# microsoft/foldingdiff

Hardware: AMD Instinct MI355X
Metric: backbones/sec (L=128, T=1000, bs=512) (higher is better)
Workload: dtype f32 (fp16 hi/lo split operands, 3x v_mfma_f32_{32x32x16,16x16x32}_f16 per product, fp32 accumulate)

## Files before the change

foldingdiff_amd/csrc/ffn16.hip:

```cpp
#include <cstdlib>
#include <type_traits>

#include "fdmi_kernels.h"
#include "img_common.h"
#include "launch_common.h"

namespace fdmi {
namespace ffn {

typedef float f32x4 __attribute__((ext_vector_type(4)));
typedef const __attribute__((address_space(3))) u32x4* lds_cu128_t;
__device__ __forceinline__ unsigned lds_addr(const void* p) { return (unsigned)(unsigned long long)(lds_ptr_t)(const_cast<void*>(p)); }
__device__ __forceinline__ u32x4 lds_u128(unsigned a) { return *(lds_cu128_t)(unsigned long long)a; }
__device__ __forceinline__ f16x8 lds_f16x8(unsigned a) { return __builtin_bit_cast(f16x8, lds_u128(a)); }

__device__ __forceinline__ void swap16(unsigned& vdst, unsigned& src) {
  const auto r = __builtin_amdgcn_permlane16_swap(vdst, src, false, false);
  vdst = r[0];
  src = r[1];
}
__device__ __forceinline__ float quad_sum(float x) {
  unsigned a = __builtin_bit_cast(unsigned, x), b = a;
  swap32(a, b);
  float m = __builtin_bit_cast(float, a) + __builtin_bit_cast(float, b);
  a = __builtin_bit_cast(unsigned, m);
  b = a;
  swap16(a, b);
  return __builtin_bit_cast(float, a) + __builtin_bit_cast(float, b);
}

template <int V> using IC = std::integral_constant<int, V>;
template <int LO, int HI, class F>
__device__ __forceinline__ void static_for(F&& f) {
  if constexpr (LO < HI) {
    f(IC<LO>{});
    static_for<LO + 1, HI>(f);
  }
}

#ifndef FDMI_FFN_DBG
#define FDMI_FFN_DBG 0
#endif
#ifndef FDMI_FFN_ST_AUX
#define FDMI_FFN_ST_AUX 0
#endif
#ifndef FDMI_FFN_PRIO
#define FDMI_FFN_PRIO 2
#endif

__device__ __forceinline__ f32x4 mfma16(const f16x8& a, const f16x8& b, const f32x4& c) {
  return __builtin_amdgcn_mfma_f32_16x16x32_f16(a, b, c, 0, 0, 0);
}

constexpr int NW = 8;
constexpr int TILE = 2048;
constexpr int STEP = 4 * TILE;
constexpr int SPS = 2;
constexpr int STAGE = SPS * STEP;
constexpr int NST = 3;
constexpr int PPW = STAGE / 1024 / NW;
constexpr int OFF_W = 0;
constexpr int OFF_X = NST * STAGE;
__host__ __device__ constexpr int off_p(int nkt) { return OFF_X + NW * nkt * 1024; }

template <int NKT, bool TAIL, bool PROF>
__global__ __launch_bounds__(64 * NW) void ffn16_kernel(FfnArgs p) {
  static_assert(NKT == 12 || NKT == 6, "d_model 384 or 192, intermediate size 2 d_model");
  constexpr int D = 32 * NKT;
  constexpr int NG = NKT;
  constexpr int SPG = 2 * NKT;
  constexpr int STG = SPG / SPS;
  static_assert(STG % NST == 0, "a group is a whole number of ring turns: its first stage always sits in slot 0");
  constexpr int NSA = TAIL ? NKT * NKT / 2 : 0;
  static_assert((NSA / SPS) % NST == 0 && NSA % SPS == 0, "whole ring turns");
  constexpr int W_BYTES = (NSA / SPS + NG * STG) * STAGE;
  constexpr int OFF_P = off_p(NKT);
  constexpr int OFF_P1 = OFF_P + 5 * D * 4;
  extern __shared__ __attribute__((aligned(16))) unsigned char smem[];
  const int tid = threadIdx.x, lane = tid & 63;
  const int wq = __builtin_amdgcn_readfirstlane(tid >> 6);
  const int grp = wq >> 2;
  unsigned smem0 = __builtin_amdgcn_readfirstlane(lds_addr(smem));
  asm volatile("" : "+s"(smem0));
  auto lane_id = [&]() __attribute__((always_inline)) {
    int ln;
    asm volatile("v_mbcnt_lo_u32_b32 %0, -1, 0\n\tv_mbcnt_hi_u32_b32 %0, -1, %0" : "=v"(ln));
    return ln;
  };
  auto lane_off_of = [](int ln) __attribute__((always_inline)) { return (unsigned)((ln >> 4) * 256 + (ln & 15) * 16); };

  {
    float* par = reinterpret_cast<float*>(smem + OFF_P);
    for (int i = tid; i < 2 * D; i += 64 * NW) par[i] = p.bi[i];
    for (int i = tid; i < D; i += 64 * NW) {
      par[2 * D + i] = p.bd[i];
      par[3 * D + i] = p.gamma[i];
      par[4 * D + i] = p.beta[i] * p.out_scale;
      if constexpr (TAIL) {
        par[5 * D + i] = p.bo[i] * (1.0f / p.ao_scale);
        par[6 * D + i] = p.g1[i];
        par[7 * D + i] = p.b1[i] * p.a_scale;
      }
    }
  }

  int w_src = 0, w_slot = 0;
  const __amdgpu_buffer_rsrc_t rs_w = __builtin_amdgcn_make_buffer_rsrc(const_cast<unsigned char*>(p.wimg), 0, W_BYTES, 0x00020000);
  auto issue_w = [&]() __attribute__((always_inline)) {
    const lds_ptr_t dst = (lds_ptr_t)(unsigned long long)(smem0 + OFF_W + (unsigned)__builtin_amdgcn_readfirstlane(w_slot));
    const int so = __builtin_amdgcn_readfirstlane(w_src);
    const int vo = lane_id() * 16;
#pragma unroll
    for (int k = 0; k < PPW; ++k) dma16(rs_w, dst + (wq + NW * k) * 1024, vo, so + (wq + NW * k) * 1024);
    w_src = w_src + STAGE == W_BYTES ? 0 : w_src + STAGE;
    w_slot = w_slot + STAGE == NST * STAGE ? 0 : w_slot + STAGE;
  };

  f16x8 ah[NKT];
  const __amdgpu_buffer_rsrc_t rs_a =
      __builtin_amdgcn_make_buffer_rsrc(const_cast<unsigned char*>(TAIL ? p.cimg : p.aimg), 0, p.a_bytes, 0x00020000);
  const __amdgpu_buffer_rsrc_t rs_h = __builtin_amdgcn_make_buffer_rsrc(const_cast<unsigned char*>(TAIL ? p.hres : p.aimg), 0, p.a_bytes, 0x00020000);
  auto row_off = [&](int r0) __attribute__((always_inline)) {
    const int ln = lane_id();
    const int row = r0 + 16 * wq + (ln & 15);
    return (unsigned)(((row >> 5) * (NKT * 256) + (row & 31)) * 16 + (ln >> 4) * 512);
  };
  u32x4 tl[NKT];
  auto load_hi = [&](int r0) __attribute__((always_inline)) {
    const unsigned hoff = row_off(r0);
#pragma unroll
    for (int kt = 0; kt < NKT; ++kt)
      ah[kt] = __builtin_bit_cast(f16x8, __builtin_amdgcn_raw_buffer_load_b128(rs_a, (int)hoff, kt * 8 * 512, 0));
  };
  auto load_lo = [&](auto KT, unsigned hoff) __attribute__((always_inline)) {
    constexpr int kt = decltype(KT)::value;
    tl[kt] = __builtin_bit_cast(u32x4, __builtin_amdgcn_raw_buffer_load_b128(rs_a, (int)hoff, (kt * 8 + 4) * 512, 0));
  };
  auto commit_lo = [&]() __attribute__((always_inline)) {
    const unsigned ax = smem0 + OFF_X + (unsigned)(wq * NKT * 1024 + lane_id() * 16);
#pragma unroll
    for (int kt = 0; kt < NKT; ++kt) *(__attribute__((address_space(3))) u32x4*)(unsigned long long)(ax + (unsigned)(kt * 1024)) = tl[kt];
  };
  const __amdgpu_buffer_rsrc_t rs_o = __builtin_amdgcn_make_buffer_rsrc(p.out, 0, p.out_bytes, 0x00020000);
  auto load_res = [&](auto KT, unsigned hoff, f32x4 (&Yr)[2 * NKT]) __attribute__((always_inline)) {
    constexpr int kt = decltype(KT)::value;
    Yr[2 * kt] = __builtin_bit_cast(f32x4, __builtin_amdgcn_raw_buffer_load_b128(rs_h, (int)hoff, kt * 8 * 512, 0));
    Yr[2 * kt + 1] = __builtin_bit_cast(f32x4, __builtin_amdgcn_raw_buffer_load_b128(rs_h, (int)hoff, (kt * 8 + 4) * 512, 0));
  };

  const bool rec = PROF && blockIdx.x == 0 && p.stamps != nullptr;
  unsigned long long* stp = PROF ? p.stamps + (size_t)wq * 16 * 16 : nullptr;
  int slot = 0;
#define FD_STAMP(i) do { if (PROF) { if (rec && slot < 16 && lane == 0) stp[slot * 16 + (i)] = __builtin_amdgcn_s_memtime(); } } while (0)
#define FD_SB() __builtin_amdgcn_sched_barrier(0)
#define FD_STAMP_G(i) do { if (PROF) { if (rec && slot == 0 && G == 1 && lane == 0) stp[15 * 16 + (i)] = __builtin_amdgcn_s_memtime(); } } while (0)

  const int n_pass = p.dims ? min(p.panels, __builtin_amdgcn_readfirstlane(p.dims[1]) >> 7) : p.panels;
  if ((int)blockIdx.x >= n_pass) return;
  const float os_up = p.up_scale, os_dn = p.down_scale, hs = 0.5f * p.g_scale;
  const f32x4 zero4 = {0.f, 0.f, 0.f, 0.f};
  f32x4 Y[2 * NKT];
  f32x4 U[4];
  f32x4 Up[4];
  u32x4 uh[2], ul[2];

  load_hi((int)blockIdx.x * 128);
  {
    const unsigned hoff = row_off((int)blockIdx.x * 128);
    static_for<0, NKT>([&](auto KT) __attribute__((always_inline)) { load_lo(KT, hoff); });
    if constexpr (TAIL) static_for<0, NKT>([&](auto KT) __attribute__((always_inline)) { load_res(KT, hoff, Y); });
  }
  issue_w();
  issue_w();
  issue_w();
  FD_WAIT_VM(3 * PPW);
  commit_lo();
  FD_WAIT_VM(2 * PPW);
  barrier_keep_vm();

  auto gelu_piece = [&](auto P, unsigned abq) __attribute__((always_inline)) {
    constexpr int pc = decltype(P)::value, pr = pc >> 2, j = pc & 3;
    const u32x2 b = *(const __attribute__((address_space(3))) u32x2*)(unsigned long long)(abq + (unsigned)((32 * pr + 2 * j) * 4));
    float o0 = __builtin_fmaf(Up[2 * pr + (j >> 1)][2 * (j & 1)], os_up, __builtin_bit_cast(float, (unsigned)b[0]));
    float o1 = __builtin_fmaf(Up[2 * pr + (j >> 1)][2 * (j & 1) + 1], os_up, __builtin_bit_cast(float, (unsigned)b[1]));
#if !(FDMI_FFN_DBG & 1)
    const float h0 = o0 * hs, h1 = o1 * hs;
    o0 = __builtin_fmaf(h0, erf_rational(o0 * 0.70710678118654752440f), h0);
    o1 = __builtin_fmaf(h1, erf_rational(o1 * 0.70710678118654752440f), h1);
#endif
    unsigned a, c;
    split_pair(o0, o1, a, c);
    uh[pr][j] = a;
    ul[pr][j] = c;
  };

  auto steps = [&](auto S0, auto S1, auto GEL, unsigned abq) __attribute__((always_inline)) {
    constexpr int s0 = decltype(S0)::value, s1 = decltype(S1)::value;
    constexpr bool gel = decltype(GEL)::value == 1, pha = decltype(GEL)::value == 2;
    auto stage_top = [&]() __attribute__((always_inline)) {
      FD_WAIT_VM(PPW);
      barrier_keep_vm();
      issue_w();
    };
    f16x8 fx[4], fy[4], xl;
    unsigned a_W, a_X;
    {
      const int ln = lane_id();
      a_W = smem0 + OFF_W + lane_off_of(ln);
      a_X = smem0 + OFF_X + (unsigned)(wq * NKT * 1024 + ln * 16);
      asm volatile("" : "+v"(a_W), "+v"(a_X));
    }
    auto plane_reads = [&](auto S, auto LO, f16x8 (&f)[4]) __attribute__((always_inline)) {
      constexpr int s = decltype(S)::value, lo = decltype(LO)::value;
      constexpr unsigned off = (unsigned)(((s / SPS) % NST) * STAGE + (s % SPS) * STEP + lo * 1024);
#if FDMI_FFN_DBG & 8
      if constexpr (lo == 1) {
#pragma unroll
        for (int t = 0; t < 4; ++t) f[t] = fx[t];
      } else
#endif
#pragma unroll
      for (int t = 0; t < 4; ++t) f[t] = lds_f16x8(a_W + off + (unsigned)(t * TILE));
      if constexpr (pha) {
        if constexpr (lo == 0 && s % (NKT / 2) == 0) xl = lds_f16x8(a_X + (unsigned)((s / (NKT / 2)) * 1024));
      } else {
        if constexpr (lo == 0 && s < NKT) xl = lds_f16x8(a_X + (unsigned)(s * 1024));
      }
    };
    auto mm = [&](auto S, auto WHICH, const f16x8 (&f)[4]) __attribute__((always_inline)) {
      constexpr int s = decltype(S)::value, which = decltype(WHICH)::value;
      if constexpr (pha) {
        constexpr int kt = s / (NKT / 2), q = s % (NKT / 2);
#pragma unroll
        for (int t = 0; t < 4; ++t) Y[4 * q + t] = mfma16(f[t], which == 1 ? xl : ah[kt], Y[4 * q + t]);
      } else if constexpr (s < NKT) {
#if !(FDMI_FFN_DBG & 4)
#pragma unroll
        for (int t = 0; t < 4; ++t) U[t] = mfma16(f[t], which == 1 ? xl : ah[s], U[t]);
#endif
      } else {
#if !(FDMI_FFN_DBG & 2)
        constexpr int pr = (s - NKT) / (NKT / 2), q = (s - NKT) % (NKT / 2);
#pragma unroll
        for (int t = 0; t < 4; ++t) Y[4 * q + t] = mfma16(f[t], __builtin_bit_cast(f16x8, which == 1 ? ul[pr] : uh[pr]), Y[4 * q + t]);
#endif
      }
    };
    plane_reads(S0, IC<0>{}, fx);
    FD_SB();
    static_for<s0, s1>([&](auto S) __attribute__((always_inline)) {
      constexpr int s = decltype(S)::value;
      constexpr bool top = s % SPS == SPS - 1;
      plane_reads(S, IC<1>{}, fy);
      FD_SB();
      if constexpr (top) {
        if (grp == 0) stage_top();
      }
#if FDMI_FFN_PRIO
      __builtin_amdgcn_s_setprio(FDMI_FFN_PRIO);
#endif
      mm(S, IC<0>{}, fx);
      mm(S, IC<1>{}, fx);
#if FDMI_FFN_PRIO
      __builtin_amdgcn_s_setprio(0);
#endif
      FD_SB();
      if constexpr (top) {
        if (grp != 0) stage_top();
      }
      if constexpr (s + 1 < s1) plane_reads(IC<s + 1>{}, IC<0>{}, fx);
      FD_SB();
      if constexpr (gel) {
        if (grp == 0) {
          static_for<0, 8>([&](auto P) __attribute__((always_inline)) {
            if constexpr (1 + decltype(P)::value * (NKT - 2) / 8 == s) gelu_piece(P, abq);
          });
        }
        FD_SB();
      }
      mm(S, IC<2>{}, fy);
      FD_SB();
      if constexpr (gel) {
        if (grp != 0) {
          static_for<0, 8>([&](auto P) __attribute__((always_inline)) {
            if constexpr (1 + decltype(P)::value * (NKT - 2) / 8 == s) gelu_piece(P, abq);
          });
        }
        FD_SB();
      }
    });
  };

  for (int panel = blockIdx.x; panel < n_pass; panel += (int)gridDim.x) {
    FD_STAMP(0);
    if constexpr (TAIL) {
      const int ln = lane_id();
      const int g = ln >> 4;
      const unsigned pb1 = smem0 + OFF_P1 + (unsigned)(8 * g * 4);
      const unsigned ax = smem0 + OFF_X + (unsigned)(wq * NKT * 1024 + ln * 16);
      {
        const float c = p.hres_inv * (1.0f / p.ao_scale);
#pragma unroll
        for (int kt = 0; kt < NKT; ++kt) {
          const u32x4 rh = __builtin_bit_cast(u32x4, Y[2 * kt]), rl = __builtin_bit_cast(u32x4, Y[2 * kt + 1]);
          const u32x4 b0 = lds_u128(pb1 + (unsigned)(kt * 128)), b1 = lds_u128(pb1 + (unsigned)(kt * 128 + 16));
#pragma unroll
          for (int j = 0; j < 2; ++j)
#pragma unroll
            for (int e = 0; e < 4; e += 2) {
              const unsigned hw = rh[2 * j + e / 2], lw = rl[2 * j + e / 2];
              const unsigned bw0 = j == 0 ? b0[e] : b1[e], bw1 = j == 0 ? b0[e + 1] : b1[e + 1];
              float v0 = fma_mix_lo(hw, c, __builtin_bit_cast(float, bw0));
              float v1 = fma_mix_hi(hw, c, __builtin_bit_cast(float, bw1));
              Y[2 * kt + j][e] = fma_mix_lo(lw, c, v0);
              Y[2 * kt + j][e + 1] = fma_mix_hi(lw, c, v1);
            }
        }
      }
      steps(IC<0>{}, IC<NSA>{}, IC<2>{}, 0u);
      const float os_ao = p.ao_scale;
      float sum = 0.f;
#pragma unroll
      for (int t = 0; t < 2 * NKT; ++t)
#pragma unroll
        for (int e = 0; e < 4; ++e) {
          Y[t][e] *= os_ao;
          sum += Y[t][e];
        }
      const float inv_n = 1.0f / (float)D;
      float mean = quad_sum(sum) * inv_n;
      asm volatile("" : "+v"(mean));
      float t2 = 0.f;
#pragma unroll
      for (int t = 0; t < 2 * NKT; ++t)
#pragma unroll
        for (int e = 0; e < 4; ++e) {
          const float dl = Y[t][e] - mean;
          Y[t][e] = dl;
          t2 = __builtin_fmaf(dl, dl, t2);
        }
      const float rstd = (1.0f / sqrtf(__builtin_fmaf(quad_sum(t2), inv_n, p.eps1))) * p.a_scale;
#pragma unroll
      for (int kt = 0; kt < NKT; ++kt) {
        const u32x4 g0 = lds_u128(pb1 + (unsigned)(D * 4 + kt * 128)), g1 = lds_u128(pb1 + (unsigned)(D * 4 + kt * 128 + 16));
        const u32x4 e0 = lds_u128(pb1 + (unsigned)(2 * D * 4 + kt * 128)), e1 = lds_u128(pb1 + (unsigned)(2 * D * 4 + kt * 128 + 16));
        float o[8];
#pragma unroll
        for (int e = 0; e < 4; ++e) {
          o[e] = __builtin_fmaf(Y[2 * kt][e] * rstd, __builtin_bit_cast(float, (unsigned)g0[e]), __builtin_bit_cast(float, (unsigned)e0[e]));
          o[4 + e] = __builtin_fmaf(Y[2 * kt + 1][e] * rstd, __builtin_bit_cast(float, (unsigned)g1[e]), __builtin_bit_cast(float, (unsigned)e1[e]));
        }
        u32x4 hv, lv;
#pragma unroll
        for (int j = 0; j < 4; ++j) {
          unsigned a, b;
          split_pair(o[2 * j], o[2 * j + 1], a, b);
          hv[j] = a;
          lv[j] = b;
        }
        ah[kt] = __builtin_bit_cast(f16x8, hv);
        *(__attribute__((address_space(3))) u32x4*)(unsigned long long)(ax + (unsigned)(kt * 1024)) = lv;
      }
    }
#pragma unroll
    for (int t = 0; t < 2 * NKT; ++t) Y[t] = zero4;
#pragma unroll
    for (int t = 0; t < 4; ++t) U[t] = zero4;
    steps(IC<0>{}, IC<NKT>{}, IC<0>{}, 0u);
    for (int G = 0; G < NG; ++G) {
#pragma unroll
      for (int t = 0; t < 4; ++t) {
        Up[t] = U[t];
        U[t] = zero4;
      }
      unsigned abq = smem0 + OFF_P + (unsigned)((64 * G + 8 * (lane_id() >> 4)) * 4);
      asm volatile("" : "+v"(abq));
      FD_STAMP_G(0);
      FD_STAMP_G(1);
      if (G + 1 < NG) {
#ifdef FDMI_FFN_NOPIPE
        static_for<0, 8>([&](auto P) __attribute__((always_inline)) { gelu_piece(P, abq); });
        steps(IC<0>{}, IC<NKT>{}, IC<0>{}, abq);
#else
        steps(IC<0>{}, IC<NKT>{}, IC<1>{}, abq);
#endif
      } else {
        static_for<0, 8>([&](auto P) __attribute__((always_inline)) { gelu_piece(P, abq); });
      }
      FD_STAMP_G(2);
      steps(IC<NKT>{}, IC<SPG>{}, IC<0>{}, 0u);
      FD_STAMP_G(3);
      if (slot == 0) FD_STAMP(1 + (G < 12 ? G : 11));
    }
    {
      const int ln = lane_id();
      const int g = ln >> 4;
      const unsigned pb = smem0 + OFF_P + (unsigned)((2 * D + 8 * g) * 4);
      const unsigned ax = smem0 + OFF_X + (unsigned)(wq * NKT * 1024 + ln * 16);
      const float ri = p.resid_inv;
      float sum = 0.f;
#pragma unroll
      for (int kt = 0; kt < NKT; ++kt) {
        const u32x4 b0 = lds_u128(pb + (unsigned)(kt * 128)), b1 = lds_u128(pb + (unsigned)(kt * 128 + 16));
        const u32x4 rh = __builtin_bit_cast(u32x4, ah[kt]), rl = lds_u128(ax + (unsigned)(kt * 1024));
#pragma unroll
        for (int j = 0; j < 2; ++j)
#pragma unroll
          for (int e = 0; e < 4; e += 2) {
            const unsigned bw0 = j == 0 ? b0[e] : b1[e], bw1 = j == 0 ? b0[e + 1] : b1[e + 1];
            float v0 = __builtin_fmaf(Y[2 * kt + j][e], os_dn, __builtin_bit_cast(float, bw0));
            float v1 = __builtin_fmaf(Y[2 * kt + j][e + 1], os_dn, __builtin_bit_cast(float, bw1));
            const unsigned hw = rh[2 * j + e / 2], lw = rl[2 * j + e / 2];
            v0 = fma_mix_lo(hw, ri, v0);
            v1 = fma_mix_hi(hw, ri, v1);
            v0 = fma_mix_lo(lw, ri, v0);
            v1 = fma_mix_hi(lw, ri, v1);
            Y[2 * kt + j][e] = v0;
            Y[2 * kt + j][e + 1] = v1;
            sum += v0;
            sum += v1;
          }
      }
      const int next = panel + (int)gridDim.x;
      load_hi(next * 128);
      const unsigned noff = row_off(next * 128);
      const float inv_n = 1.0f / (float)D;
      float mean = quad_sum(sum) * inv_n;
      asm volatile("" : "+v"(mean));
      float t2 = 0.f;
#pragma unroll
      for (int t = 0; t < 2 * NKT; ++t)
#pragma unroll
        for (int e = 0; e < 4; ++e) {
          const float dl = Y[t][e] - mean;
          Y[t][e] = dl;
          t2 = __builtin_fmaf(dl, dl, t2);
        }
      const float rstd = (1.0f / sqrtf(__builtin_fmaf(quad_sum(t2), inv_n, p.eps))) * p.out_scale;
      const unsigned ooff = row_off(panel * 128);
      static_for<0, NKT>([&](auto KT) __attribute__((always_inline)) {
        constexpr int kt = decltype(KT)::value;
        const u32x4 g0 = lds_u128(pb + (unsigned)(D * 4 + kt * 128)), g1 = lds_u128(pb + (unsigned)(D * 4 + kt * 128 + 16));
        const u32x4 e0 = lds_u128(pb + (unsigned)(2 * D * 4 + kt * 128)), e1 = lds_u128(pb + (unsigned)(2 * D * 4 + kt * 128 + 16));
        float o[8];
#pragma unroll
        for (int e = 0; e < 4; ++e) {
          o[e] = __builtin_fmaf(Y[2 * kt][e] * rstd, __builtin_bit_cast(float, (unsigned)g0[e]), __builtin_bit_cast(float, (unsigned)e0[e]));
          o[4 + e] = __builtin_fmaf(Y[2 * kt + 1][e] * rstd, __builtin_bit_cast(float, (unsigned)g1[e]), __builtin_bit_cast(float, (unsigned)e1[e]));
        }
        u32x4 hv, lv;
#pragma unroll
        for (int j = 0; j < 4; ++j) {
          unsigned a, b;
          split_pair(o[2 * j], o[2 * j + 1], a, b);
          hv[j] = a;
          lv[j] = b;
        }
#if FDMI_FFN_DBG & 16
        if (hv[0] == 0x12345678u && lv[1] == 0x9abcdef0u)
#endif
        {
          __builtin_amdgcn_raw_buffer_store_b128(hv, rs_o, (int)ooff, kt * 8 * 512, FDMI_FFN_ST_AUX);
          __builtin_amdgcn_raw_buffer_store_b128(lv, rs_o, (int)ooff, (kt * 8 + 4) * 512, FDMI_FFN_ST_AUX);
        }
        load_lo(KT, noff);
        if constexpr (TAIL) load_res(KT, noff, Y);
        FD_SB();
      });
    }
    FD_STAMP(13);
    FD_WAIT_VM(0);
    commit_lo();
    FD_STAMP(14);
    ++slot;
  }
  FD_WAIT_VM(0);
#undef FD_STAMP
#undef FD_STAMP_G
#undef FD_SB
}

template <int NKT, bool TAIL>
static bool launch(const FfnArgs& p, hipStream_t s) {
  constexpr int SMEM = off_p(NKT) + (TAIL ? 8 : 5) * 32 * NKT * 4;
  static LdsOptIn lds;
  if (!lds({reinterpret_cast<const void*>(&ffn16_kernel<NKT, TAIL, false>), reinterpret_cast<const void*>(&ffn16_kernel<NKT, TAIL, true>)}, SMEM))
    return false;
  int grid = cu_count();
  if (grid > p.panels) grid = p.panels;
  if (grid <= 0) return true;
  if (p.stamps) hipLaunchKernelGGL((ffn16_kernel<NKT, TAIL, true>), dim3(grid), dim3(64 * NW), SMEM, s, p);
  else hipLaunchKernelGGL((ffn16_kernel<NKT, TAIL, false>), dim3(grid), dim3(64 * NW), SMEM, s, p);
  return hipGetLastError() == hipSuccess;
}

}

bool ffn16_supported(int d_model, int d_ff) { return (d_model == 384 || d_model == 192) && d_ff == 2 * d_model; }

bool launch_ffn16(const FfnArgs& p, int d_model, hipStream_t s) {
  if (p.cimg) return d_model == 384 ? ffn::launch<12, true>(p, s) : ffn::launch<6, true>(p, s);
  return d_model == 384 ? ffn::launch<12, false>(p, s) : ffn::launch<6, false>(p, s);
}

}
```

Measured before the change: 78.95.

## Interleave LayerNorm apply into first up-projection steps and fold ao_scale into eps

When the tail (attention-output) path is active, the LayerNorm normalise/affine/split of the residual is no longer done as a separate loop. Only the first two k-tiles are done up front, and the rest are computed inside the first up-projection step sequence, interleaved with the MFMA work and split between wave groups. The ao_scale multiply on the accumulators is removed by folding it into a rescaled epsilon. This is meant to hide the LN VALU work behind matrix ops. It adds register pressure and relies on the scale folding being numerically equivalent.

```diff
diff --git a/foldingdiff_amd/csrc/ffn16.hip b/foldingdiff_amd/csrc/ffn16.hip
--- a/foldingdiff_amd/csrc/ffn16.hip
+++ b/foldingdiff_amd/csrc/ffn16.hip
@@ -46,6 +46,9 @@
 #endif
 #ifndef FDMI_FFN_PRIO
 #define FDMI_FFN_PRIO 2
+#endif
+#ifndef FDMI_FFN_PHASES
+#define FDMI_FFN_PHASES 1
 #endif
 
 __device__ __forceinline__ f32x4 mfma16(const f16x8& a, const f16x8& b, const f32x4& c) {
@@ -76,6 +79,7 @@
   constexpr int W_BYTES = (NSA / SPS + NG * STG) * STAGE;
   constexpr int OFF_P = off_p(NKT);
   constexpr int OFF_P1 = OFF_P + 5 * D * 4;
+  constexpr bool FOLD = TAIL && FDMI_FFN_PHASES != 0;
   extern __shared__ __attribute__((aligned(16))) unsigned char smem[];
   const int tid = threadIdx.x, lane = tid & 63;
   const int wq = __builtin_amdgcn_readfirstlane(tid >> 6);
@@ -153,11 +157,15 @@
   int slot = 0;
 #define FD_STAMP(i) do { if (PROF) { if (rec && slot < 16 && lane == 0) stp[slot * 16 + (i)] = __builtin_amdgcn_s_memtime(); } } while (0)
 #define FD_SB() __builtin_amdgcn_sched_barrier(0)
+#define FD_STAMP_U(k) do { if (PROF) { if (rec && slot < 15 && lane == 0) stp[slot == 0 ? 15 * 16 + 4 + (k) : slot * 16 + 1 + (k)] = __builtin_amdgcn_s_memtime(); } } while (0)
 #define FD_STAMP_G(i) do { if (PROF) { if (rec && slot == 0 && G == 1 && lane == 0) stp[15 * 16 + (i)] = __builtin_amdgcn_s_memtime(); } } while (0)
 
   const int n_pass = p.dims ? min(p.panels, __builtin_amdgcn_readfirstlane(p.dims[1]) >> 7) : p.panels;
   if ((int)blockIdx.x >= n_pass) return;
   const float os_up = p.up_scale, os_dn = p.down_scale, hs = 0.5f * p.g_scale;
+  const float eps1_raw = FOLD ? __builtin_bit_cast(float, __builtin_amdgcn_readfirstlane(__builtin_bit_cast(
+                                    int, (p.eps1 * (1.0f / p.ao_scale)) * (1.0f / p.ao_scale)))) : p.eps1;
+  float rstd1 = 0.f;
   const f32x4 zero4 = {0.f, 0.f, 0.f, 0.f};
   f32x4 Y[2 * NKT];
   f32x4 U[4];
@@ -194,9 +202,33 @@
     ul[pr][j] = c;
   };
 
+  auto ln_piece = [&](auto KT, unsigned pq, unsigned ax) __attribute__((always_inline)) {
+    constexpr int kt = decltype(KT)::value;
+    u32x4 hv, lv;
+    static_for<0, 2>([&](auto J) __attribute__((always_inline)) {
+      constexpr int j = decltype(J)::value;
+      const u32x4 gm = lds_u128(pq + (unsigned)(6 * D * 4 + kt * 128 + 16 * j)), bt = lds_u128(pq + (unsigned)(7 * D * 4 + kt * 128 + 16 * j));
+      float o[4];
+#pragma unroll
+      for (int e = 0; e < 4; ++e)
+        o[e] = __builtin_fmaf(Y[2 * kt + j][e] * rstd1, __builtin_bit_cast(float, (unsigned)gm[e]), __builtin_bit_cast(float, (unsigned)bt[e]));
+      Y[2 * kt + j] = zero4;
+#pragma unroll
+      for (int q = 0; q < 2; ++q) {
+        unsigned a, b;
+        split_pair(o[2 * q], o[2 * q + 1], a, b);
+        hv[2 * j + q] = a;
+        lv[2 * j + q] = b;
+      }
+      if constexpr (j == 0) FD_SB();
+    });
+    ah[kt] = __builtin_bit_cast(f16x8, hv);
+    *(__attribute__((address_space(3))) u32x4*)(unsigned long long)(ax + (unsigned)(kt * 1024)) = lv;
+  };
+
   auto steps = [&](auto S0, auto S1, auto GEL, unsigned abq) __attribute__((always_inline)) {
     constexpr int s0 = decltype(S0)::value, s1 = decltype(S1)::value;
-    constexpr bool gel = decltype(GEL)::value == 1, pha = decltype(GEL)::value == 2;
+    constexpr bool gel = decltype(GEL)::value == 1, pha = decltype(GEL)::value == 2, lnp = decltype(GEL)::value == 3;
     auto stage_top = [&]() __attribute__((always_inline)) {
       FD_WAIT_VM(PPW);
       barrier_keep_vm();
@@ -278,8 +310,16 @@
         }
         FD_SB();
       }
+      if constexpr (lnp && s + 2 < NKT) {
+        if (grp == 0) ln_piece(IC<s + 2>{}, abq, a_X);
+        FD_SB();
+      }
       mm(S, IC<2>{}, fy);
       FD_SB();
+      if constexpr (lnp && s + 2 < NKT) {
+        if (grp != 0) ln_piece(IC<s + 2>{}, abq, a_X);
+        FD_SB();
+      }
       if constexpr (gel) {
         if (grp != 0) {
           static_for<0, 8>([&](auto P) __attribute__((always_inline)) {
@@ -318,13 +358,14 @@
         }
       }
       steps(IC<0>{}, IC<NSA>{}, IC<2>{}, 0u);
+      FD_STAMP(15);
       const float os_ao = p.ao_scale;
       float sum = 0.f;
 #pragma unroll
       for (int t = 0; t < 2 * NKT; ++t)
 #pragma unroll
         for (int e = 0; e < 4; ++e) {
-          Y[t][e] *= os_ao;
+          if constexpr (!FOLD) Y[t][e] *= os_ao;
           sum += Y[t][e];
         }
       const float inv_n = 1.0f / (float)D;
@@ -339,7 +380,9 @@
           Y[t][e] = dl;
           t2 = __builtin_fmaf(dl, dl, t2);
         }
-      const float rstd = (1.0f / sqrtf(__builtin_fmaf(quad_sum(t2), inv_n, p.eps1))) * p.a_scale;
+      const float rstd = (1.0f / sqrtf(__builtin_fmaf(quad_sum(t2), inv_n, eps1_raw))) * p.a_scale;
+      rstd1 = rstd;
+      if constexpr (!FOLD) {
 #pragma unroll
       for (int kt = 0; kt < NKT; ++kt) {
         const u32x4 g0 = lds_u128(pb1 + (unsigned)(D * 4 + kt * 128)), g1 = lds_u128(pb1 + (unsigned)(D * 4 + kt * 128 + 16));
@@ -361,12 +404,30 @@
         ah[kt] = __builtin_bit_cast(f16x8, hv);
         *(__attribute__((address_space(3))) u32x4*)(unsigned long long)(ax + (unsigned)(kt * 1024)) = lv;
       }
-    }
-#pragma unroll
-    for (int t = 0; t < 2 * NKT; ++t) Y[t] = zero4;
+      }
+    }
+    if constexpr (!FOLD) {
+#pragma unroll
+      for (int t = 0; t < 2 * NKT; ++t) Y[t] = zero4;
+    }
 #pragma unroll
     for (int t = 0; t < 4; ++t) U[t] = zero4;
-    steps(IC<0>{}, IC<NKT>{}, IC<0>{}, 0u);
+    if constexpr (FOLD) {
+      const int ln = lane_id();
+      unsigned pq = smem0 + OFF_P + (unsigned)(8 * (ln >> 4) * 4);
+      const unsigned ax = smem0 + OFF_X + (unsigned)(wq * NKT * 1024 + ln * 16);
+      asm volatile("" : "+v"(pq));
+      ln_piece(IC<0>{}, pq, ax);
+      ln_piece(IC<1>{}, pq, ax);
+#pragma unroll
+      for (int kt = 2; kt < NKT; ++kt) ah[kt] = ah[0];
+      FD_STAMP_U(0);
+      steps(IC<0>{}, IC<NKT>{}, IC<3>{}, pq);
+    } else {
+      FD_STAMP_U(0);
+      steps(IC<0>{}, IC<NKT>{}, IC<0>{}, 0u);
+    }
+    FD_STAMP_U(1);
     for (int G = 0; G < NG; ++G) {
 #pragma unroll
       for (int t = 0; t < 4; ++t) {
@@ -390,7 +451,7 @@
       FD_STAMP_G(2);
       steps(IC<NKT>{}, IC<SPG>{}, IC<0>{}, 0u);
       FD_STAMP_G(3);
-      if (slot == 0) FD_STAMP(1 + (G < 12 ? G : 11));
+      if (slot == 0 || G == NG - 1) FD_STAMP(1 + (G < 12 ? G : 11));
     }
     {
       const int ln = lane_id();
@@ -477,6 +538,7 @@
   FD_WAIT_VM(0);
 #undef FD_STAMP
 #undef FD_STAMP_G
+#undef FD_STAMP_U
 #undef FD_SB
 }
 
```

Result: no change. 78.93 (median of 2 runs) (-0.0%).
